# MILAB-IIT-CV/ATDN_vSLAM

Hardware: AMD Instinct MI355X
Metric: frame-pairs/sec, KITTI 1241x376 odometry inference at 1/2/4/8 MI355X (higher is better)
Workload: dtype f32 via 3xf16 split MFMA (fp32 accumulate); 1 GPU; KITTI seq-03-shaped 376x1241 uint8 frames (resident in HBM) resized to 376x1232, GMA flow 12 GRU iters + CLVO head -> 6-DoF trajectory (BASELINE configs[1]); streams_per_gpu=2, gru_iters=12, parallelism=pairs sharded x1, one all-gather of 512-d features, replicated LSTM scan

## Files before the change

### atdn_vslam_amd/csrc/gma.h

```cpp
#pragma once
#include <vector>
#include <map>
#include <memory>

#include "attention.h"
#include "conv_dispatch.h"
#include "device_buf.h"
#include "kernels.h"
#include "range_probe.h"
#include "weights.h"

namespace atdn {

struct EncoderWeights {
  PackedConv stem;
  struct Block { PackedConv c1, c2, ds; bool has_ds = false; } blk[6];
  PackedConv head;
};

class GmaNet {
 public:
  GmaNet(int H, int W, int max_batch, int precision);
  ~GmaNet();
  StateDict& state() { return sd_; }
// ... 11 lines not shown
  void profile(int B, int iters, int reps, float* ms, hipStream_t st, int mode = 0);

  int H, W, H8, W8, N, ldN, maxB, precision;
  int dev_ = 0;
  bool norm_on_load_ = false;
  bool classic_ = false;
  bool low_latency_ = false;
  void set_low_latency(bool on);
  DeviceBuf attn_part_;
  DeviceBuf enc2_[4];
  hipStream_t par_stream_ = nullptr;
  std::vector<hipEvent_t> par_events_;
  size_t par_next_ = 0;
  bool par_ = false;
  bool par_ok_ = true;
  void fork(hipStream_t from, hipStream_t to);
  DeviceBuf fbrick_[4], fplain_[3], coords_used_;
  DeviceBuf fpre_, fsrc_;
  PackedConv fhead_fold_;
  float corr_mul_ = 1.f;
  long fhead_w32_off_ = -1, fhead_b32_off_ = -1;
  int brickBW_[4], brickBH_[4], brickNB_[4];
  BrickPyramid brick_pyramid() const;
  DeviceBuf rowmax_, rinv_;

  struct ProbeRow { std::string name; int iter; bool limited; float max_abs; long long over, nonfinite; };
  static constexpr int kProbeMaxRows = 1536;
  void set_probe(bool on);
  const std::vector<ProbeRow>& probe_rows() const { return probe_rows_; }

 private:
  bool probe_ = false;
  int probe_it_ = -1;
  DeviceArray<RangeSlot> probe_slots_;
  std::vector<ProbeRow> probe_rows_;
  void probe_begin(hipStream_t st);
  void probe_end(hipStream_t st);
  void probe(const std::string& name, bool limited, const float* p, long rows, long cols, long ld, hipStream_t st);
  void run_body(int B, int iters, hipStream_t st);
  void run_encoder(const EncoderWeights& E, bool instance, int nimg, hipStream_t st, float** out_buf, int* outH,
                   int* outW);
  void iteration(int B, hipStream_t st);
  void run_body_sf(int B, int iters, hipStream_t st);
  void run_encoder_sf(const EncoderWeights& E, bool instance, int nimg, hipStream_t st, float** out_buf, int first_img = 0,
                      DeviceBuf* bufs = nullptr, float* final_dst = nullptr);
  void iteration_sf(int B, hipStream_t st);
  void capture(int B, int iters);
  void launch_body(int B, int iters, hipStream_t st);
  int seq_ = 0;
  int last_frame_ = -1;
  float* preds_out_ = nullptr;
  long preds_stride_ = 0;
  void mask_head_sf(int B, hipStream_t st);
  void mask_head(int B, hipStream_t st);
  int last_B_ = 0;

  StateDict sd_;
  WeightArena arena_;
  bool ready_ = false;
  bool use_graph_ = true;
  EncoderWeights fnet_, cnet_;
  PackedConv convc1_, convc2_, convf1_, convf2_, convm_, to_v_, to_qk_;
  long convf1_sf_off_ = -1;
  float convf1_wscale_ = 1.f;
  float fh2_mul_ = 1.f;
  long fh2_w32_off_ = -1;
  DeviceBuf fhG_;
  PackedConv gru_zr_[2], gru_q_[2], fh1_, fh2_, mask0_, mask2_;
  PackedConv gru_zr_ctx_[2], gru_q_ctx_[2];
  const float* gamma_ = nullptr;
  long gamma_off_ = -1;
  long to_v_w32_off_ = -1;

  DeviceBuf img4_, enc_[4], scratch_, pcnt_, fin_, fmap_ , psum_, pm2_, mean_[3], rstd_[3];
  DeviceBuf pyr_[4], h_[2], x_, qk_, attn_, vT_, corrfeat_, cor1_, corflo_, flo1_, z_, rh_, fh_, mask_;
  DeviceBuf coords1_, flow4_, pre_zr_[2], pre_q_[2];
  int pyrH_[4], pyrW_[4];
  size_t ws_bytes_ = 0;

  struct Timer;
  Timer* timer_ = nullptr;
  void mark(int stage, hipStream_t st);

  hipStream_t cap_stream_ = nullptr;
  std::map<std::pair<int, int>, hipGraphExec_t> graphs_;
};

}
```

### atdn_vslam_amd/csrc/gma.hip

```cpp
#include "gma.h"
#include "small_convs.h"
#include "conv_sf.h"
#include "epilogues_sf.h"

namespace atdn { const float* zero_line(); }

namespace atdn {

extern template TileChoice conv_dispatch<MODE_TAP, EpiBias<ACT_NONE>>(const ConvShape&, EpiBias<ACT_NONE>, hipStream_t);
extern template TileChoice conv_dispatch<MODE_TAP, EpiBias<ACT_RELU>>(const ConvShape&, EpiBias<ACT_RELU>, hipStream_t);
extern template TileChoice conv_dispatch<MODE_ROW, EpiBias<ACT_RELU>>(const ConvShape&, EpiBias<ACT_RELU>, hipStream_t);
extern template TileChoice conv_dispatch<MODE_TAP, EpiBiasStats>(const ConvShape&, EpiBiasStats, hipStream_t);
extern template TileChoice conv_dispatch<MODE_ROW, EpiBiasStats>(const ConvShape&, EpiBiasStats, hipStream_t);
extern template TileChoice conv_dispatch<MODE_TAP, EpiBiasReluAddRelu>(const ConvShape&, EpiBiasReluAddRelu, hipStream_t);
extern template TileChoice conv_dispatch<MODE_TAP, EpiContextSplit>(const ConvShape&, EpiContextSplit, hipStream_t);
extern template TileChoice conv_dispatch<MODE_TAP, EpiScale>(const ConvShape&, EpiScale, hipStream_t);
extern template TileChoice conv_dispatch<MODE_TAP, EpiQK>(const ConvShape&, EpiQK, hipStream_t);
extern template TileChoice conv_dispatch<MODE_TAP, EpiStoreT>(const ConvShape&, EpiStoreT, hipStream_t);
extern template TileChoice conv_dispatch<MODE_TAP, EpiAggregate>(const ConvShape&, EpiAggregate, hipStream_t);
extern template TileChoice conv_dispatch<MODE_TAP, EpiGruZR>(const ConvShape&, EpiGruZR, hipStream_t);
extern template TileChoice conv_dispatch<MODE_TAP, EpiGruQ>(const ConvShape&, EpiGruQ, hipStream_t);
extern template TileChoice conv_dispatch<MODE_TAP, EpiFlowDelta>(const ConvShape&, EpiFlowDelta, hipStream_t);

extern template TileChoice conv_dispatch<MODE_ROW, SfBias<ACT_RELU>>(const ConvShape&, SfBias<ACT_RELU>, hipStream_t);
// ... 202 lines not shown
    convf1_sf_off_ = arena_.alloc(4L * 2 * 4 * 2 * 64 * 4);
    _Float16* f = reinterpret_cast<_Float16*>(arena_.at(convf1_sf_off_));
    for (int wv = 0; wv < 4; ++wv)
      for (int cb = 0; cb < 2; ++cb)
        for (int s = 0; s < 4; ++s)
          for (int lane = 0; lane < 64; ++lane)
            for (int i = 0; i < 8; ++i) {
              const int n = 32 * wv + 16 * cb + (lane & 15), g = lane >> 4;
              const int ky = 2 * s + (g >> 1), kx = 4 * (g & 1) + (i >> 1), c = i & 1;
              const float v = (ky < 7 && kx < 7) ? std::ldexp(w.data[(((long)n * 2 + c) * 7 + ky) * 7 + kx], p) : 0.f;
              const _Float16 hi = (_Float16)v, lo = (_Float16)(v - (float)hi);
              const long frag = (((long)wv * 2 + cb) * 4 + s) * 2;
              f[(frag * 64 + lane) * 8 + i] = hi;
              f[((frag + 1) * 64 + lane) * 8 + i] = lo;
            }
  }
  convf2_ = tap({u + "encoder.convf2"});
  convm_ = tap({u + "encoder.conv"});
  to_v_ = tap({u + "aggregator.to_v"}, false);
  to_qk_ = tap({"att.to_qk"}, false);
  for (int p = 0; p < 2; ++p) {
    const std::string t = std::to_string(p + 1);
    if (sf) {
      const std::vector<std::pair<int, int>> ctx = {{128, 256}};
      const HostTensor& wv = sd_.get(u + "aggregator.to_v.weight");
      const HostTensor& gam = sd_.get(u + "aggregator.gamma");
      ATDN_CHECK(gam.data.size() == 1, "aggregator.gamma is one value");
      gru_zr_[p] = pack_gru_sf_folded(arena_, sd_, {u + "gru.convz" + t, u + "gru.convr" + t}, wv, (double)gam.data[0]);
      gru_q_[p] = pack_gru_sf_folded(arena_, sd_, {u + "gru.convq" + t}, wv, (double)gam.data[0]);
      gru_zr_ctx_[p] = pack_conv_sf_channels(arena_, sd_, {u + "gru.convz" + t, u + "gru.convr" + t}, ctx, false);
      gru_q_ctx_[p] = pack_conv_sf_channels(arena_, sd_, {u + "gru.convq" + t}, ctx, false);
    } else {
      gru_zr_[p] = tap({u + "gru.convz" + t, u + "gru.convr" + t});
      gru_q_[p] = tap({u + "gru.convq" + t});
    }
  }
  fh1_ = tap({u + "flow_head.conv1"});
  fh2_ = tap({u + "flow_head.conv2"});
  if (sf) {
    const HostTensor& w = sd_.get(u + "flow_head.conv2.weight");
    ATDN_CHECK(w.shape.size() == 4 && w.shape[0] == 2 && w.shape[1] == 256 && w.shape[2] == 3 && w.shape[3] == 3, "flow head conv2 shape");
    fh2_w32_off_ = arena_.alloc(18 * 256);
    for (int o = 0; o < 2; ++o)
      for (int c = 0; c < 256; ++c)
        for (int t = 0; t < 9; ++t) arena_.at(fh2_w32_off_)[(t * 2 + o) * 256 + c] = w.data[((long)o * 256 + c) * 9 + t];
    float mx = 0.f;
    for (float v : w.data) mx = std::max(mx, std::fabs(v));
    int e = 0;
    if (mx > 0.f) (void)std::frexp(mx, &e);
    fh2_mul_ = std::ldexp(1.0f, 1 - e);
  }
  mask0_ = tap({u + "mask.0"});
  mask2_ = tap({u + "mask.2"});
  gamma_off_ = pack_vector(arena_, sd_.get(u + "aggregator.gamma").data);
  if (sf) to_v_w32_off_ = pack_vector(arena_, sd_.get(u + "aggregator.to_v.weight").data);
  arena_.upload();
  resolve_encoder(arena_, fnet_);
  resolve_encoder(arena_, cnet_);
  for (PackedConv* L : {&convc1_, &convc2_, &convf1_, &convf2_, &convm_, &to_v_, &to_qk_, &gru_zr_[0], &gru_zr_[1],
                        &gru_q_[0], &gru_q_[1], &fh1_, &fh2_, &mask0_, &mask2_})
    resolve(arena_, *L);
  if (sf) for (PackedConv* L : {&gru_zr_ctx_[0], &gru_zr_ctx_[1], &gru_q_ctx_[0], &gru_q_ctx_[1], &fhead_fold_}) resolve(arena_, *L);
  gamma_ = arena_.dev(gamma_off_);

  const int B = maxB;
  const int H2 = conv_out(H, 7, 2, 3), W2 = conv_out(W, 7, 2, 3);
  const long n8 = (long)B * N;
  img4_.alloc(2L * B * H * W * 4);
  for (int i = 0; i < (sf ? 4 : 3); ++i) enc_[i].alloc(2L * B * H2 * W2 * 64);
  if (sf) { fpre_.alloc(2L * B * N * 128); fsrc_.alloc((long)B * N * 160); }
  else fmap_.alloc(2L * B * N * 256);
  const long groups = (long)cdiv(H2 * W2, 64) * 4 + 8;
  psum_.alloc(2L * B * groups * 128); pm2_.alloc(2L * B * groups * 128); pcnt_.alloc(2L * B * groups); fin_.alloc(2L * B * 32 * 128 * 4 * 2);
  for (int i = 0; i < 3; ++i) { mean_[i].alloc(2L * B * 128); rstd_[i].alloc(2L * B * 128); }
  pyrH_[0] = H8; pyrW_[0] = W8;
  for (int l = 1; l < 4; ++l) { pyrH_[l] = pyrH_[l - 1] / 2; pyrW_[l] = pyrW_[l - 1] / 2; }
  ATDN_CHECK(pyrH_[3] >= 2 && pyrW_[3] >= 2, "frame too small for a 4-level pyramid");
  for (int l = 0; l < 4; ++l) {
    brickBW_[l] = cdiv(pyrW_[l], 8); brickBH_[l] = cdiv(pyrH_[l], 4); brickNB_[l] = brickBW_[l] * brickBH_[l] * 32;
    pyr_[l].alloc(classic_ ? n8 * pyrH_[l] * pyrW_[l] : (long)B * brick_pixel_blocks(N) * kBrickPixelBlock * brickNB_[l]);
  }
  if (sf) {
    for (int l = 0; l < 4; ++l) fbrick_[l].alloc((long)B * brickNB_[l] * 160);
    for (int l = 1; l < 4; ++l) fplain_[l - 1].alloc((long)B * pyrH_[l] * pyrW_[l] * 128);
    coords_used_.alloc(n8 * 2);
  }
  h_[0].alloc(n8 * 128); h_[1].alloc(n8 * 128); x_.alloc(n8 * XLD);
  const AttnGeom ag = attn_geom(B, N, ldN);
  qk_.alloc(n8 * 256); attn_.alloc(std::max(n8 * ldN, attn_floats(ag)));
  if (classic_) vT_.alloc((long)B * 128 * ldN);
  if (sf) { rowmax_.alloc((long)B * ag.Npad); rinv_.alloc((long)B * ag.Npad); }
  if (sf && low_latency_ && attn_v_splits(attn_geom(1, N, ldN)) > 1) attn_part_.alloc(8L * B * ag.Npad * 128);
  if (sf && low_latency_) {
    for (int i = 0; i < 4; ++i) enc2_[i].alloc((long)B * H2 * W2 * 64);
    ATDN_HIP(hipStreamCreateWithFlags(&par_stream_, hipStreamNonBlocking));
    par_events_.resize(2 * (1 + 64));
    for (auto& e : par_events_) ATDN_HIP(hipEventCreateWithFlags(&e, hipEventDisableTiming));
  }
  corrfeat_.alloc(n8 * CORR_LD); cor1_.alloc(n8 * 256); corflo_.alloc(n8 * 256); flo1_.alloc(n8 * 128);
  z_.alloc(n8 * 128); rh_.alloc(n8 * 128); fh_.alloc(n8 * 256); mask_.alloc(n8 * 576);
  if (sf) fhG_.alloc(2 * n8 * 18);
  coords1_.alloc(n8 * 2); flow4_.alloc(n8 * 4);
  if (sf) for (int p = 0; p < 2; ++p) { pre_zr_[p].alloc(n8 * 256); pre_q_[p].alloc(n8 * 128); }
  ATDN_HIP(hipMemset(corrfeat_.p, 0, corrfeat_.n * sizeof(float)));
  if (vT_.p) ATDN_HIP(hipMemset(vT_.p, 0, vT_.n * sizeof(float)));
  ATDN_HIP(hipMemset(attn_.p, 0, attn_.n * sizeof(float)));
  ATDN_HIP(hipMemset(flow4_.p, 0, flow4_.n * sizeof(float)));
  ATDN_HIP(hipDeviceSynchronize());
  ws_bytes_ = 0;
  DeviceBuf* all[] = {&img4_, &enc_[0], &enc_[1], &enc_[2], &enc_[3], &fmap_, &fpre_, &fsrc_, &psum_, &pm2_, &pyr_[0], &pyr_[1], &pyr_[2],
                      &pyr_[3], &h_[0], &h_[1], &x_, &qk_, &attn_, &vT_, &corrfeat_, &cor1_, &corflo_, &flo1_, &z_,
                      &rh_, &fh_, &mask_, &coords1_, &flow4_};
  for (auto* b : all) ws_bytes_ += (size_t)b->n * sizeof(float);
  (void)zero_line();
  sf_counter_attach();
  ATDN_HIP(hipStreamCreateWithFlags(&cap_stream_, hipStreamNonBlocking));
  ready_ = true;
}

void GmaNet::run_encoder(const EncoderWeights& E, bool instance, int nimg, hipStream_t st, float** out_buf, int* outH,
                         int* outW) {
  int h = conv_out(H, 7, 2, 3), w = conv_out(W, 7, 2, 3);
  float* P = enc_[0].p; float* Q = enc_[1].p; float* R = enc_[2].p;
  auto stats_conv = [&](auto mode_tag, const PackedConv& L, const float* src, int ld, int ih, int iw, int stride,
                        int pad, float* dst, int slot) {
    constexpr int MODE = decltype(mode_tag)::value;
    ConvShape s = conv_shape(L, src, ld, (long)ih * iw * ld, nimg, ih, iw, stride, pad, pad);
    const int oh = conv_out(ih, L.KH, stride, pad), ow = conv_out(iw, L.KW, stride, pad);
    EpiBiasStats ep{L.b, dst, (long)oh * ow * L.N, L.N, psum_.p, pm2_.p, 0};
    TileChoice t = conv_dispatch<MODE>(s, ep, st);
    const int groups = cdiv(oh * ow, t.BM) * (t.BM / 32);
    ATDN_CHECK((long)nimg * groups * L.N <= psum_.n, "statistics scratch too small");
    launch_in_finalize_cnt(psum_.p, pm2_.p, nullptr, nimg, groups, oh * ow, L.N, 1e-5f, mean_[slot].p, rstd_[slot].p,
                           reinterpret_cast<double*>(fin_.p), st);
  };
  using TapT = std::integral_constant<int, MODE_TAP>;
  using RowT = std::integral_constant<int, MODE_ROW>;
  auto pr = [&](int bi, const char* leaf, bool limited, const float* p, long pixels, int ch) {
    if (!probe_) return;
    std::string name = instance ? "fnet." : "cnet.";
    if (bi >= 0) name += "layer" + std::to_string(bi / 2 + 1) + "." + std::to_string(bi % 2);
    probe(name + leaf, limited, p, (long)nimg * pixels, ch, ch, st);
  };

  if (instance) {
    stats_conv(RowT{}, E.stem, img4_.p, 4, H, W, 2, 3, P, 0);
    pr(-1, "conv1.raw", false, P, (long)h * w, 64);
    launch_in_apply(P, mean_[0].p, rstd_[0].p, nullptr, nullptr, nullptr, nimg, (long)h * w, 64, st);
  } else {
    ConvShape s = conv_shape(E.stem, img4_.p, 4, (long)H * W * 4, nimg, H, W, 2, 3, 3);
    conv_dispatch<MODE_ROW>(s, EpiBias<ACT_RELU>{E.stem.b, P, (long)h * w * 64, 64, 1.f}, st);
  }
  pr(-1, "conv1.out", true, P, (long)h * w, 64);
// ... 324 lines not shown
  run_encoder_sf(fnet_, true, nfeat, st, &f, seq_ == 2 ? 1 : 0, nullptr, fpre_.p + (seq_ == 2 ? (long)N * 128 : 0));
  ConvShape s = conv_shape(fhead_fold_, fpre_.p, 128, (long)N * 128, B, H8, W8, 1, 0, 0);
  conv_sf_dispatch(s, fhead_fold_.wscale, SfBias<ACT_NONE>{fhead_fold_.b, fsrc_.p, (long)N * 160, 160}, st);
  mark(ST_FNET, st);

  const float* target = fpre_.p + (long)(seq_ ? 1 : B) * N * 128;
  for (int l = 0; l < 4; ++l) {
    const float* plain = target;
    long plain_sb = (long)N * 128;
    if (l > 0) {
      const float* prev = l == 1 ? target : fplain_[l - 2].p;
      const long prev_sb = l == 1 ? (long)N * 128 : (long)pyrH_[l - 1] * pyrW_[l - 1] * 128;
      plain_sb = (long)pyrH_[l] * pyrW_[l] * 128;
      launch_pool_features_sf(prev, B, pyrH_[l - 1], pyrW_[l - 1], 128, prev_sb, fplain_[l - 1].p, plain_sb, st);
      plain = fplain_[l - 1].p;
    }
    launch_brick_rows(plain, plain_sb, B, pyrH_[l], pyrW_[l], 128, 160, fbrick_[l].p, (long)brickNB_[l] * 160, st);
    launch_corr_bricks(fsrc_.p, (long)N * 160, fbrick_[l].p, (long)brickNB_[l] * 160, B, N, brickNB_[l], 160,
                       corr_mul_ / sqrtf(256.0f), pyr_[l].p, sf_fast_mode(), st);
    if (l == 0) mark(ST_CORR, st);
  }
  mark(ST_POOL, st);

  run_encoder_sf(cnet_, false, B, sB, &f, 0, par_ ? enc2_ : nullptr);
  s = conv_shape(cnet_.head, f, 128, (long)N * 128, B, H8, W8, 1, 0, 0);
  conv_sf_dispatch(s, cnet_.head.wscale,
                   SfContextSplit{cnet_.head.b, h_[0].p, (long)N * 128, x_.p, (long)N * XLD, XLD}, sB);
  mark(ST_CNET, st);

  s = conv_shape(to_qk_, x_.p, XLD, (long)N * XLD, B, H8, W8, 1, 0, 0);
  conv_sf_dispatch(s, to_qk_.wscale, SfQK{1.0f / sqrtf(128.0f), 128, qk_.p, (long)N * 256, 256}, sB);
  {
    const AttnGeom ag = attn_geom(B, N, ldN);
    launch_qk_rowmax(qk_.p, ag, rowmax_.p, sB);
    mark(ST_ATTN_LOGITS, st);
    launch_qk_softmax(qk_.p, ag, rowmax_.p, attn_.p, rinv_.p, sf_fast_mode(), sB);
  }
  mark(ST_ATTN, st);

  for (int p = 0; p < 2; ++p) {
    const int ph = p ? 2 : 0, pw = p ? 0 : 2;
    ConvShape g = conv_shape(gru_zr_ctx_[p], x_.p, XLD, (long)N * XLD, B, H8, W8, 1, ph, pw);
    conv_sf_dispatch(g, gru_zr_ctx_[p].wscale, EpiBias<ACT_NONE>{nullptr, pre_zr_[p].p, (long)N * 256, 256, 1.f}, sB);
    g = conv_shape(gru_q_ctx_[p], x_.p, XLD, (long)N * XLD, B, H8, W8, 1, ph, pw);
    conv_sf_dispatch(g, gru_q_ctx_[p].wscale, EpiBias<ACT_NONE>{nullptr, pre_q_[p].p, (long)N * 128, 128, 1.f}, sB);
  }
  mark(ST_GRU_CTX, st);
  if (par_) fork(sB, st);

  for (int it = 0; it < iters; ++it) {
    iteration_sf(B, st);
    if (preds_out_) {
      mask_head_sf(B, st);
      launch_upsample(mask_.p, flow4_.p, B, H8, W8, nullptr, preds_out_ + it * preds_stride_, st);
    }
  }
  if (!preds_out_) mask_head_sf(B, st);
  mark(ST_MASK, st);
}

void GmaNet::mask_head_sf(int B, hipStream_t st) {
  ConvShape s = conv_shape(mask0_, h_[0].p, 128, (long)N * 128, B, H8, W8, 1, 1, 1);
  conv_sf_dispatch(s, mask0_.wscale, SfBias<ACT_RELU>{mask0_.b, fh_.p, (long)N * 256, 256}, st);
  s = conv_shape(mask2_, fh_.p, 256, (long)N * 256, B, H8, W8, 1, 0, 0);
  conv_sf_dispatch(s, mask2_.wscale, EpiBias<ACT_NONE>{mask2_.b, mask_.p, (long)N * 576, 576, 0.25f}, st);
}

void GmaNet::capture(int B, int iters) {
  const bool want_par = low_latency_ && precision >= 1 && B <= 2 && par_stream_ != nullptr && !preds_out_ && par_ok_;
  for (int attempt = want_par ? 0 : 1; attempt < 2; ++attempt) {
    hipGraph_t graph = nullptr;
    hipGraphExec_t exec = nullptr;
    ATDN_HIP(hipStreamBeginCapture(cap_stream_, hipStreamCaptureModeThreadLocal));
    par_ = attempt == 0;
    par_next_ = 0;
    try {
      if (precision >= 1) { FastGuard fg(precision == 2); run_body_sf(B, iters, cap_stream_); } else run_body(B, iters, cap_stream_);
      par_ = false;
      ATDN_HIP(hipStreamEndCapture(cap_stream_, &graph));
      ATDN_HIP(hipGraphInstantiate(&exec, graph, nullptr, nullptr, 0));
    } catch (...) {
      const bool was_par = par_ || attempt == 0;
      par_ = false;
      hipGraph_t g2 = nullptr;
      (void)hipStreamEndCapture(cap_stream_, &g2);
      if (g2) (void)hipGraphDestroy(g2);
      if (graph) (void)hipGraphDestroy(graph);
      (void)hipGetLastError();
      if (attempt == 0 && was_par) {
        fprintf(stderr, "atdn: the flow graph could not be captured with parallel branches; capturing it as one chain\n");
        par_ok_ = false;
        continue;
      }
      throw;
    }
    (void)hipGraphDestroy(graph);
    graphs_[{B, iters * 4 + seq_}] = exec;
    return;
  }
}

void GmaNet::forward_sequence(const float* frames, int B, int iters, const float* flow_init, float* flow_low,
                               float* flow_up, hipStream_t st, bool continued) {
  ATDN_CHECK(ready_, "weights not finalized");
  ATDN_CHECK(precision >= 1, "sequence mode is built for the split-f16 pipeline");
  ATDN_CHECK(B >= 1 && B <= maxB, "batch exceeds max_batch of this handle");
  ATDN_CHECK(iters >= 1 && iters <= 64, "iters out of range");
  ATDN_CHECK(frames && flow_low && flow_up, "null tensor");
  const long frame = 3L * H * W;
  if (continued) {
    ATDN_CHECK(last_frame_ >= 1, "continued sequence call without a previous sequence call on this handle");
    ATDN_HIP(hipMemcpyAsync(fpre_.p, fpre_.p + (long)last_frame_ * N * 128, (size_t)N * 128 * sizeof(float),
                            hipMemcpyDeviceToDevice, st));
    seq_ = 2;
  } else {
    seq_ = 1;
  }
  last_frame_ = 0;
  launch_prep_images(frames, frames + (long)B * frame, B, H, W, img4_.p, st, 1);
  launch_init_coords_sf(flow_init, B, H8, W8, coords1_.p, flow4_.p, x_.p, XLD, 254, st);
  launch_body(B, iters, st);
  launch_upsample(mask_.p, flow4_.p, B, H8, W8, flow_low, flow_up, st);
  last_frame_ = B;
}

void GmaNet::launch_body(int B, int iters, hipStream_t st) {
  last_B_ = B;
  if (use_graph_ && !probe_) {
    auto key = std::make_pair(B, iters * 4 + seq_);
    if (!graphs_.count(key)) capture(B, iters);
    ATDN_HIP(hipGraphLaunch(graphs_[key], st));
  } else {
    if (precision >= 1) { FastGuard fg(precision == 2); run_body_sf(B, iters, st); } else run_body(B, iters, st);
  }
}

void GmaNet::forward(const float* im1, const float* im2, int B, int iters, const float* flow_init, float* flow_low,
                     float* flow_up, hipStream_t st) {
  ATDN_CHECK(ready_, "weights not finalized");
  ATDN_CHECK(B >= 1 && B <= maxB, "batch exceeds max_batch of this handle");
  ATDN_CHECK(iters >= 1 && iters <= 64, "iters out of range");
  ATDN_CHECK(im1 && im2 && flow_low && flow_up, "null tensor");
  seq_ = 0;
  last_frame_ = 0;
  if (probe_) probe_begin(st);
  launch_prep_images(im1, im2, B, H, W, img4_.p, st, B);
  if (precision >= 1) launch_init_coords_sf(flow_init, B, H8, W8, coords1_.p, flow4_.p, x_.p, XLD, 254, st);
  else launch_init_coords(flow_init, B, H8, W8, coords1_.p, flow4_.p, x_.p + 254, XLD, st);
  if (probe_) {
    probe("image", true, img4_.p, 2L * B * H * W, 3, 4, st);
    probe("flow_init", true, flow4_.p, (long)B * N, 2, 4, st);
  }
  launch_body(B, iters, st);
  launch_upsample(mask_.p, flow4_.p, B, H8, W8, flow_low, flow_up, st);
  if (probe_) {
    probe("flow_low", false, flow_low, 1, 2L * B * N, 2L * B * N, st);
    probe("flow_up", false, flow_up, 1, 2L * B * H * W, 2L * B * H * W, st);
    probe_end(st);
  }
}

void GmaNet::forward_predictions(const float* im1, const float* im2, int B, int iters, const float* flow_init, float* preds,
                                 hipStream_t st) {
  ATDN_CHECK(ready_, "weights not finalized");
  ATDN_CHECK(B >= 1 && B <= maxB, "batch exceeds max_batch of this handle");
  ATDN_CHECK(iters >= 1 && iters <= 64, "iters out of range");
  ATDN_CHECK(im1 && im2 && preds, "null tensor");
  seq_ = 0;
  last_frame_ = 0;
  last_B_ = B;
  if (probe_) probe_begin(st);
  launch_prep_images(im1, im2, B, H, W, img4_.p, st, B);
  if (precision >= 1) launch_init_coords_sf(flow_init, B, H8, W8, coords1_.p, flow4_.p, x_.p, XLD, 254, st);
  else launch_init_coords(flow_init, B, H8, W8, coords1_.p, flow4_.p, x_.p + 254, XLD, st);
  if (probe_) {
    probe("image", true, img4_.p, 2L * B * H * W, 3, 4, st);
    probe("flow_init", true, flow4_.p, (long)B * N, 2, 4, st);
  }
  struct Guard {
    GmaNet* n; ~Guard() { n->preds_out_ = nullptr; n->preds_stride_ = 0; }
  } guard{this};
  preds_out_ = preds;
  preds_stride_ = (long)B * 2 * H * W;
  if (precision >= 1) { FastGuard fg(precision == 2); run_body_sf(B, iters, st); } else run_body(B, iters, st);
  if (probe_) probe_end(st);
}

BrickPyramid GmaNet::brick_pyramid() const {
  BrickPyramid bp;
  for (int l = 0; l < 4; ++l) {
    bp.base[l] = pyr_[l].p; bp.H[l] = pyrH_[l]; bp.W[l] = pyrW_[l];
    bp.BW[l] = brickBW_[l]; bp.BH[l] = brickBH_[l]; bp.NB[l] = brickNB_[l];
  }
  bp.N = N; bp.NPB = brick_pixel_blocks(N);
  return bp;
}

long GmaNet::debug_read(const char* name, float* host, long capacity, hipStream_t st) {
  const std::string k(name);
  if (!classic_ && k.size() == 4 && k.compare(0, 3, "pyr") == 0 && k[3] >= '0' && k[3] <= '3') {
    const int l = k[3] - '0';
    const long rows = (long)maxB * N, total = rows * pyrH_[l] * pyrW_[l];
    scratch_.reserve(total);
    launch_unbrick(pyr_[l].p, brickNB_[l], N, pyrH_[l], pyrW_[l], rows, scratch_.p, st);
    ATDN_HIP(hipStreamSynchronize(st));
    const long n = std::min(capacity, total);
    ATDN_HIP(hipMemcpy(host, scratch_.p, (size_t)n * sizeof(float), hipMemcpyDeviceToHost));
    return n;
  }
  if (!classic_ && k == "corrfeat") {
    launch_lookup_bricks(brick_pyramid(), coords_used_.p, (long)(last_B_ > 0 ? last_B_ : maxB) * N, corrfeat_.p, st);
  }
  if (k == "sf_clamped") {
    ATDN_CHECK(capacity >= 1, "sf_clamped needs room for one float");
    host[0] = (float)sf_counter_read_reset(st);
    return 1;
  }
  const DeviceBuf* b = nullptr;
  if (k == "fmap") b = &fmap_; else if (k == "pyr0") b = &pyr_[0]; else if (k == "pyr1") b = &pyr_[1];
  else if (k == "pyr2") b = &pyr_[2]; else if (k == "pyr3") b = &pyr_[3]; else if (k == "net") b = &h_[0];
  else if (k == "x") b = &x_; else if (k == "attn") b = &attn_; else if (k == "corrfeat") b = &corrfeat_;
  else if (k == "mask") b = &mask_; else if (k == "coords1") b = &coords1_; else if (k == "flow4") b = &flow4_;
  else if (k == "qk") b = &qk_; else if (k == "img4") b = &img4_;
  else if (k == "cor1") b = &cor1_;
  if (k == "fmap" && !classic_) {
    const long rows = 2L * maxB * N;
    scratch_.reserve(rows * (128 + 256));
    launch_from_sf(fpre_.p, scratch_.p, rows, 128, st);
    launch_linear_rows(scratch_.p, rows, 128, arena_.dev(fhead_w32_off_), arena_.dev(fhead_b32_off_), 256, scratch_.p + rows * 128, st);
    ATDN_HIP(hipStreamSynchronize(st));
    const long n = std::min(capacity, rows * 256);
    ATDN_HIP(hipMemcpy(host, scratch_.p + rows * 128, (size_t)n * sizeof(float), hipMemcpyDeviceToHost));
    return n;
  }
  if (k == "agg") {
    if (classic_) return -1;
    scratch_.reserve(x_.n);
    launch_from_sf(x_.p, scratch_.p, x_.n / 32, 32, st);
    ATDN_HIP(hipStreamSynchronize(st));
    const long rows = std::min(capacity / 128, (long)maxB * N);
    if (rows > 0)
      ATDN_HIP(hipMemcpy2D(host, 128 * sizeof(float), scratch_.p + 256, XLD * sizeof(float), 128 * sizeof(float), (size_t)rows,
                           hipMemcpyDeviceToHost));
    return rows * 128;
  }
  if (!b) return -1;
  long n = std::min(capacity, b->n);
  if (k == "attn" && !classic_) {
    const long rows = (long)maxB * N * ldN;
    scratch_.reserve(rows);
    ATDN_HIP(hipMemsetAsync(scratch_.p, 0, (size_t)rows * sizeof(float), st));
    launch_attn_decode(attn_.p, rinv_.p, attn_geom(maxB, N, ldN), scratch_.p, st);
    ATDN_HIP(hipStreamSynchronize(st));
    n = std::min(capacity, rows);
    ATDN_HIP(hipMemcpy(host, scratch_.p, (size_t)n * sizeof(float), hipMemcpyDeviceToHost));
    return n;
  }
  const bool is_sf = precision >= 1 && (k == "fmap" || k == "net" || k == "x" || k == "attn" || k == "corrfeat" || k == "qk" || k == "cor1");
  const float* src = b->p;
  if (is_sf) {
    scratch_.reserve(b->n);
    launch_from_sf(b->p, scratch_.p, b->n / 32, 32, st);
    src = scratch_.p;
    if (k == "x")
      launch_mfg_reconstruct(scratch_.p, (long)maxB * N, XLD, 128, 256, arena_.dev(to_v_w32_off_), gamma_, coords_used_.p, N, W8, 254, st);
// ... 8 lines not shown
```

### atdn_vslam_amd/csrc/kernels.h

```cpp
#pragma once
#include "common.h"

namespace atdn {

bool& sf_fast_mode();

struct PyramidLevels {
  const float* base[4];
  int H[4], W[4];
};

void launch_prep_images(const float* im1, const float* im2, int B, int H, int W, float* img4, hipStream_t st, int n2);

int stem_sf_groups(int Ho, int Wo);
void launch_stem_sf(int mode, const float* img4, int nimg, int H, int W, const float* wfrag, float wscale,
                    const float* bias, float* out_sf, float* part_sum, float* part_m2, float* part_cnt,
                    const float* mean, const float* rstd, hipStream_t st);

void launch_in_finalize_cnt(const float* part_sum, const float* part_m2, const float* part_cnt, int nimg,
                            int groups_per_img, int HW, int C, float eps, float* mean, float* rstd, double* scratch,
                            hipStream_t st);
void launch_in_apply(float* x, const float* mean, const float* rstd, const float* res, const float* rmean,
                     const float* rrstd, int nimg, long HW, int C, hipStream_t st);

void launch_avgpool(const float* src, int H, int W, float* dst, long rows, hipStream_t st);

void launch_lookup(const PyramidLevels& pyr, const float* coords1, long npix_total, float* out, int ldo,
                   hipStream_t st);

void launch_softmax_rows(float* x, long rows, int n, int ld, hipStream_t st);

void launch_init_coords(const float* flow_init, int B, int H8, int W8, float* coords1, float* flow4, float* xflow,
                        int ldx, hipStream_t st);

void launch_upsample(const float* mask, const float* flow4, int B, int H8, int W8, float* flow_low, float* flow_up,
                     hipStream_t st);

void launch_prep_flow(const float* flow, int B, int H, int W, const float* dw_w, const float* dw_b, float* out4,
                      hipStream_t st);
void launch_prep_rgb(const float* images, int B, int H, int W, float* out4, hipStream_t st);
void launch_linear(const float* W0, const float* x0, int K0, int ldx0, const float* W1, const float* x1, int K1,
                   int ldx1, const float* b0, const float* b1, int act, float* y, int ldy, int N, int B,
                   hipStream_t st);
struct LstmPipeArgs {
  int Hd, B, do1, do_lin, do2;
  const float *pre1, *Whh1, *bhh1, *h1_in; float *c1, *h1_out;
  const float *Wlin, *blin, *lin_in; float* lin_out;
  const float *Wih2, *bih2, *Whh2, *bhh2, *x2_in, *h2_in; float *c2, *h2_out;
};
void launch_lstm_pipe(const LstmPipeArgs& a, hipStream_t st);
long lstm_scan_exchange_bytes();
bool lstm_scan_fits_device();
void launch_lstm_scan(const float* pre1, const float* Whh1, const float* bhh1, const float* Wlin, const float* blin,
                      const float* Wih2, const float* bih2, const float* Whh2, const float* bhh2, float* state, float* h2seq,
                      void* exchange, int T, hipStream_t st);
struct MlpHead { const float *w0, *b0, *w1, *b1, *w2; };
void launch_mlp_heads(const float* h2, int B, MlpHead rot, MlpHead tr, float* rot_out, float* tr_out, hipStream_t st);

void launch_to_sf(const float* src, float* dst, long rows, int C, hipStream_t st);
void launch_from_sf(const float* src, float* dst, long rows, int C, hipStream_t st);
void launch_mfg_reconstruct(float* x, long rows, int ld, int cmf, int cagg, const float* wv, const float* gamma,
                            const float* coords_used, int N, int W8, int cflow, hipStream_t st);
void launch_in_apply_sf(const float* x, float* y, const float* mean, const float* rstd, const float* res,
                        const float* res_raw, const float* rmean, const float* rrstd, int nimg, long HW, int C,
                        hipStream_t st, bool res_relu = false);
void launch_pool_features_sf(const float* src, int nimg, int H, int W, int C, long sb, float* dst, long db, hipStream_t st);
void launch_init_coords_sf(const float* flow_init, int B, int H8, int W8, float* coords1, float* flow4, float* x,
                           int ldx, int cflow, hipStream_t st);

void launch_fill(float* p, long n, float v, hipStream_t st);

constexpr int kBrickPixelBlock = 64;
struct BrickPyramid {
  const float* base[4];
  int H[4], W[4], BW[4], BH[4], NB[4];
  int N;
  int NPB;
};
inline int brick_pixel_blocks(int N) { return 2 * ((N + 127) / 128); }
void launch_brick_rows(const float* src, long sb, int nimg, int H, int W, int C, int Cd, float* dst, long db, hipStream_t st);
void launch_corr_bricks(const float* f1, long sb1, const float* f2b, long sb2, int B, int N, int NB, int K, float scale,
                        float* out, bool fast, hipStream_t st);
void launch_linear_rows(const float* in, long rows, int Cin, const float* w, const float* b, int Cout, float* out, hipStream_t st);
void launch_unbrick(const float* src, long NB, int N, int H, int W, long npix, float* dst, hipStream_t st);
void launch_lookup_conv(const BrickPyramid& pyr, const float* coords1, long npix, float* coords_used, const float* wfrag,
                        float wscale, const float* bias, float* out, bool fast, hipStream_t st);
void launch_lookup_bricks(const BrickPyramid& pyr, const float* coords1, long npix, float* out, hipStream_t st);

}
// ... 1 lines not shown
```

### atdn_vslam_amd/csrc/weights.h

```cpp
#pragma once
#include <algorithm>
#include <cmath>
#include <cstring>
#include <map>
#include <string>
#include <vector>

#include "conv_mfma.h"
#include "device_buf.h"

namespace atdn {

struct HostTensor {
  std::vector<int64_t> shape;
  std::vector<float> data;
  long numel() const { long n = 1; for (auto d : shape) n *= d; return n; }
};

class StateDict {
 public:
  void put(const std::string& key, const float* data, const int64_t* shape, int rank) {
    std::string k = key;
    if (k.rfind("module.", 0) == 0) k = k.substr(7);
    HostTensor t;
// ... 74 lines not shown
  ATDN_CHECK(w0.shape.size() == 4, "conv weight must be 4-d");
  const int Cin = (int)w0.shape[1], KH = (int)w0.shape[2], KW = (int)w0.shape[3];
  L.mode = mode; L.KH = KH; L.KW = KW;
  L.C = (mode == MODE_TAP) ? round_up(Cin, 32) : Cpix;
  ATDN_CHECK(L.C >= Cin, "channel padding smaller than Cin");
  L.ldw = packed_k(mode, KH, KW, L.C);
  int N = 0;
  for (auto& nm : names) N += (int)sd.get(nm + ".weight").shape[0];
  L.N = N;
  L.w_off = A.alloc((long)N * L.ldw);
  L.b_off = A.alloc(N);
  int n0 = 0;
  for (auto& nm : names) {
    const HostTensor& w = sd.get(nm + ".weight");
    ATDN_CHECK((int)w.shape[1] == Cin && (int)w.shape[2] == KH && (int)w.shape[3] == KW, "stacked convs must agree");
    const int Co = (int)w.shape[0];
    const float* bias = (has_bias && sd.has(nm + ".bias")) ? sd.get(nm + ".bias").data.data() : nullptr;
    for (int n = 0; n < Co; ++n) {
      const double sc = fold ? fold->scale[n0 + n] : 1.0;
      float* row = A.at(L.w_off + (long)(n0 + n) * L.ldw);
      for (int c = 0; c < Cin; ++c)
        for (int ky = 0; ky < KH; ++ky)
          for (int kx = 0; kx < KW; ++kx) {
            const double v = (double)w.data[(((long)n * Cin + c) * KH + ky) * KW + kx] * sc;
            const long k = (mode == MODE_TAP) ? ((long)(ky * KW + kx) * L.C + c)
                                              : ((long)ky * round_up(KW * L.C, 32) + kx * L.C + c);
            row[k] = (float)v;
          }
      double bv = bias ? (double)bias[n] : 0.0;
      if (fold) bv = bv * sc + fold->shift[n0 + n];
      A.at(L.b_off)[n0 + n] = (float)bv;
    }
    n0 += Co;
  }
  return L;
}

inline void pack_fragment_major16(WeightArena& A, PackedConv& L) {
  const int nq = L.ldw / 32, nblk = (L.N + 15) / 16;
  L.wf16_off = A.alloc((long)nblk * nq * 512);
  const float* w = A.at(L.w_off);
  float* f = A.at(L.wf16_off);
  for (int nb = 0; nb < nblk; ++nb)
    for (int q = 0; q < nq; ++q)
      for (int hl = 0; hl < 2; ++hl)
        for (int lane = 0; lane < 64; ++lane) {
          const int r = lane & 15, gq = lane >> 4, row = nb * 16 + r, slot = 4 * hl + gq;
          float* d = f + ((((long)nb * nq + q) * 2 + hl) * 64 + lane) * 4;
          if (row < L.N) std::memcpy(d, w + (long)row * L.ldw + q * 32 + slot * 4, 16);
          else std::memset(d, 0, 16);
        }
}

inline PackedConv pack_conv_sf(WeightArena& A, const StateDict& sd, const std::vector<std::string>& names,
                               const ChannelAffine* fold = nullptr, bool has_bias = true) {
  PackedConv L = pack_conv(A, sd, names, MODE_TAP, 0, fold, has_bias);
  float* w = A.at(L.w_off);
  const long total = (long)L.N * L.ldw;
  float mx = 0.f;
  for (long i = 0; i < total; ++i) mx = std::max(mx, std::fabs(w[i]));
  int e = 0;
  if (mx > 0.f) (void)std::frexp(mx, &e);
  const int p = 1 - e;
  L.wscale = std::ldexp(1.0f, -p);
  std::vector<float> row(L.ldw);
  for (int n = 0; n < L.N; ++n) {
    float* r = w + (long)n * L.ldw;
    std::memcpy(row.data(), r, L.ldw * sizeof(float));
    _Float16* hrow = reinterpret_cast<_Float16*>(r);
    for (int q = 0; q < L.ldw / 32; ++q)
      for (int j = 0; j < 32; ++j) {
        const float v = std::ldexp(row[q * 32 + j], p);
        const _Float16 hi = (_Float16)v;
        const _Float16 lo = (_Float16)(v - (float)hi);
        hrow[q * 64 + j] = hi;
        hrow[q * 64 + 32 + j] = lo;
      }
  }
  if ((L.KH == 3 && L.KW == 3) || (L.KH == 1 && L.KW == 5) || (L.KH == 5 && L.KW == 1)) {
    pack_fragment_major16(A, L);
  }
  return L;
}

inline void pack_stem_sf(WeightArena& A, PackedConv& L) {
  ATDN_CHECK(L.mode == MODE_ROW && L.KH == 7 && L.KW == 7 && L.C == 4 && L.ldw == 224 && L.N == 64, "stem shape");
  L.wf_off = A.alloc(2L * 14 * 2 * 256);
  const float* w = A.at(L.w_off);
  float mx = 0.f;
  for (long i = 0; i < (long)L.N * L.ldw; ++i) mx = std::max(mx, std::fabs(w[i]));
  int e = 0;
  if (mx > 0.f) (void)std::frexp(mx, &e);
  const int p = 1 - e;
  L.wscale = std::ldexp(1.0f, -p);
  _Float16* f = reinterpret_cast<_Float16*>(A.at(L.wf_off));
  for (int nt = 0; nt < 2; ++nt)
    for (int q = 0; q < 14; ++q)
      for (int lane = 0; lane < 64; ++lane) {
        const int r = lane & 31, h = lane >> 5;
        for (int m = 0; m < 8; ++m) {
          const float v = std::ldexp(w[(long)(nt * 32 + r) * L.ldw + 16 * q + 8 * h + m], p);
          const _Float16 hi = (_Float16)v;
          f[(((long)(nt * 14 + q) * 2 + 0) * 64 + lane) * 8 + m] = hi;
          f[(((long)(nt * 14 + q) * 2 + 1) * 64 + lane) * 8 + m] = (_Float16)(v - (float)hi);
        }
      }
// ... 133 lines not shown
```

Before: 447.6 frame-pairs/s.

## Fuse mask conv2 with convex upsampling into one MFMA kernel

Replaces the separate 1x1 mask.2 conv (which wrote a 576-channel mask to HBM) and the upsample kernel with a single kernel. It computes the mask logits via split-f16 MFMA in registers, applies the softmax over the 9 neighbours, and writes the upsampled flow directly. This removes the large mask write and read and one launch per forward. The cost is a bespoke kernel with heavy register use and special weight packing, and debug reads now recompute the stored mask on demand.

```diff
diff --git a/atdn_vslam_amd/csrc/gma.h b/atdn_vslam_amd/csrc/gma.h
--- a/atdn_vslam_amd/csrc/gma.h
+++ b/atdn_vslam_amd/csrc/gma.h
@@ -87,6 +87,8 @@
   float* preds_out_ = nullptr;
   long preds_stride_ = 0;
   void mask_head_sf(int B, hipStream_t st);
+  void upsample_sf(int B, float* flow_low, float* flow_up, hipStream_t st);
+  void mask2_stored_sf(int B, float* dst, hipStream_t st);
   void mask_head(int B, hipStream_t st);
   int last_B_ = 0;
 
diff --git a/atdn_vslam_amd/csrc/gma.hip b/atdn_vslam_amd/csrc/gma.hip
--- a/atdn_vslam_amd/csrc/gma.hip
+++ b/atdn_vslam_amd/csrc/gma.hip
@@ -278,6 +278,7 @@
   }
   mask0_ = tap({u + "mask.0"});
   mask2_ = tap({u + "mask.2"});
+  if (sf) pack_mask_upsample_fragments(arena_, mask2_);
   gamma_off_ = pack_vector(arena_, sd_.get(u + "aggregator.gamma").data);
   if (sf) to_v_w32_off_ = pack_vector(arena_, sd_.get(u + "aggregator.to_v.weight").data);
   arena_.upload();
@@ -324,7 +325,8 @@
     for (auto& e : par_events_) ATDN_HIP(hipEventCreateWithFlags(&e, hipEventDisableTiming));
   }
   corrfeat_.alloc(n8 * CORR_LD); cor1_.alloc(n8 * 256); corflo_.alloc(n8 * 256); flo1_.alloc(n8 * 128);
-  z_.alloc(n8 * 128); rh_.alloc(n8 * 128); fh_.alloc(n8 * 256); mask_.alloc(n8 * 576);
+  z_.alloc(n8 * 128); rh_.alloc(n8 * 128); fh_.alloc(n8 * 256);
+  if (classic_) mask_.alloc(n8 * 576);
   if (sf) fhG_.alloc(2 * n8 * 18);
   coords1_.alloc(n8 * 2); flow4_.alloc(n8 * 4);
   if (sf) for (int p = 0; p < 2; ++p) { pre_zr_[p].alloc(n8 * 256); pre_q_[p].alloc(n8 * 128); }
@@ -755,7 +757,7 @@
     iteration_sf(B, st);
     if (preds_out_) {
       mask_head_sf(B, st);
-      launch_upsample(mask_.p, flow4_.p, B, H8, W8, nullptr, preds_out_ + it * preds_stride_, st);
+      upsample_sf(B, nullptr, preds_out_ + it * preds_stride_, st);
     }
   }
   if (!preds_out_) mask_head_sf(B, st);
@@ -765,8 +767,16 @@
 void GmaNet::mask_head_sf(int B, hipStream_t st) {
   ConvShape s = conv_shape(mask0_, h_[0].p, 128, (long)N * 128, B, H8, W8, 1, 1, 1);
   conv_sf_dispatch(s, mask0_.wscale, SfBias<ACT_RELU>{mask0_.b, fh_.p, (long)N * 256, 256}, st);
-  s = conv_shape(mask2_, fh_.p, 256, (long)N * 256, B, H8, W8, 1, 0, 0);
-  conv_sf_dispatch(s, mask2_.wscale, EpiBias<ACT_NONE>{mask2_.b, mask_.p, (long)N * 576, 576, 0.25f}, st);
+}
+
+void GmaNet::upsample_sf(int B, float* flow_low, float* flow_up, hipStream_t st) {
+  launch_mask_upsample(fh_.p, mask2_.wf16, mask2_.wscale, mask2_.b, flow4_.p, B, H8, W8, flow_low, flow_up, precision == 2, st);
+}
+
+void GmaNet::mask2_stored_sf(int B, float* dst, hipStream_t st) {
+  FastGuard fg(precision == 2);
+  ConvShape s = conv_shape(mask2_, fh_.p, 256, (long)N * 256, B, H8, W8, 1, 0, 0);
+  conv_sf_dispatch(s, mask2_.wscale, EpiBias<ACT_NONE>{mask2_.b, dst, (long)N * 576, 576, 0.25f}, st);
 }
 
 void GmaNet::capture(int B, int iters) {
@@ -823,7 +833,7 @@
   launch_prep_images(frames, frames + (long)B * frame, B, H, W, img4_.p, st, 1);
   launch_init_coords_sf(flow_init, B, H8, W8, coords1_.p, flow4_.p, x_.p, XLD, 254, st);
   launch_body(B, iters, st);
-  launch_upsample(mask_.p, flow4_.p, B, H8, W8, flow_low, flow_up, st);
+  upsample_sf(B, flow_low, flow_up, st);
   last_frame_ = B;
 }
 
@@ -855,7 +865,8 @@
     probe("flow_init", true, flow4_.p, (long)B * N, 2, 4, st);
   }
   launch_body(B, iters, st);
-  launch_upsample(mask_.p, flow4_.p, B, H8, W8, flow_low, flow_up, st);
+  if (classic_) launch_upsample(mask_.p, flow4_.p, B, H8, W8, flow_low, flow_up, st);
+  else upsample_sf(B, flow_low, flow_up, st);
   if (probe_) {
     probe("flow_low", false, flow_low, 1, 2L * B * N, 2L * B * N, st);
     probe("flow_up", false, flow_up, 1, 2L * B * H * W, 2L * B * H * W, st);
@@ -914,6 +925,24 @@
   if (!classic_ && k == "corrfeat") {
     launch_lookup_bricks(brick_pyramid(), coords_used_.p, (long)(last_B_ > 0 ? last_B_ : maxB) * N, corrfeat_.p, st);
   }
+  if (!classic_ && (k == "mask" || k == "flow_up_stored" || k == "flow_low_stored")) {
+    const int Bl = last_B_ > 0 ? last_B_ : maxB;
+    const long nmask = (long)maxB * N * 576, nup = (long)Bl * 2 * H * W, nlow = (long)Bl * 2 * N;
+    scratch_.reserve(nmask + nup + nlow);
+    ATDN_HIP(hipMemsetAsync(scratch_.p, 0, (size_t)nmask * sizeof(float), st));
+    mask2_stored_sf(Bl, scratch_.p, st);
+    const float* src = scratch_.p;
+    long total = nmask;
+    if (k != "mask") {
+      launch_upsample(scratch_.p, flow4_.p, Bl, H8, W8, scratch_.p + nmask + nup, scratch_.p + nmask, st);
+      src = k == "flow_up_stored" ? scratch_.p + nmask : scratch_.p + nmask + nup;
+      total = k == "flow_up_stored" ? nup : nlow;
+    }
+    ATDN_HIP(hipStreamSynchronize(st));
+    const long n = std::min(capacity, total);
+    ATDN_HIP(hipMemcpy(host, src, (size_t)n * sizeof(float), hipMemcpyDeviceToHost));
+    return n;
+  }
   if (k == "sf_clamped") {
     ATDN_CHECK(capacity >= 1, "sf_clamped needs room for one float");
     host[0] = (float)sf_counter_read_reset(st);
diff --git a/atdn_vslam_amd/csrc/kernels.h b/atdn_vslam_amd/csrc/kernels.h
--- a/atdn_vslam_amd/csrc/kernels.h
+++ b/atdn_vslam_amd/csrc/kernels.h
@@ -35,6 +35,8 @@
 
 void launch_upsample(const float* mask, const float* flow4, int B, int H8, int W8, float* flow_low, float* flow_up,
                      hipStream_t st);
+void launch_mask_upsample(const float* fh, const float* wfrag, float wscale, const float* bias, const float* flow4, int B,
+                          int H8, int W8, float* flow_low, float* flow_up, bool fast, hipStream_t st);
 
 void launch_prep_flow(const float* flow, int B, int H, int W, const float* dw_w, const float* dw_b, float* out4,
                       hipStream_t st);
diff --git a/atdn_vslam_amd/csrc/mask_upsample.hip b/atdn_vslam_amd/csrc/mask_upsample.hip
--- /dev/null
+++ b/atdn_vslam_amd/csrc/mask_upsample.hip
@@ -0,0 +1,201 @@
+#include "kernels.h"
+#include "sf.h"
+
+namespace atdn {
+
+namespace {
+
+constexpr int MU_NWM = 2;
+constexpr int MU_PIX = 64 * MU_NWM;
+constexpr int MU_THREADS = 256 * MU_NWM;
+constexpr int MU_ROWF = 40;
+constexpr int MU_IMG = MU_PIX * MU_ROWF;
+constexpr int MU_SLAB = 2 * MU_IMG / (4 * MU_NWM);
+constexpr int MU_PLANE = 264;
+static_assert(4 * MU_PLANE <= MU_SLAB, "a half-wave's four planes fit its slab");
+
+typedef float f32x4v __attribute__((ext_vector_type(4)));
+
+template <bool FAST>
+__global__ __launch_bounds__(MU_THREADS) void mask_upsample_kernel(const float* __restrict__ fh, const float* __restrict__ wfrag,
+                                                                   const float wscale, const float* __restrict__ bias,
+                                                                   const float* __restrict__ flow4, const int H8, const int W8,
+                                                                   const int tiles, float* __restrict__ flow_low,
+                                                                   float* __restrict__ flow_up) {
+  extern __shared__ __attribute__((aligned(16))) float lds[];
+  const int tid = threadIdx.x, lane = tid & 63, wave = tid >> 6;
+  const int wm = wave >> 2, wg = wave & 3;
+  const int N = H8 * W8;
+  const int img = blockIdx.x / tiles;
+  const int pix0 = (blockIdx.x - img * tiles) * MU_PIX;
+  const float4* f4 = reinterpret_cast<const float4*>(flow4) + (long)img * N;
+
+  if (flow_low && tid < MU_PIX && pix0 + tid < N) {
+    const float4 f = f4[pix0 + tid];
+    flow_low[((long)img * 2 + 0) * N + pix0 + tid] = f.x;
+    flow_low[((long)img * 2 + 1) * N + pix0 + tid] = f.y;
+  }
+
+  const int SL = MU_PIX + 2 * W8 + 2;
+  float2* strip = reinterpret_cast<float2*>(lds + 2 * MU_IMG);
+  for (int idx = tid; idx < SL; idx += MU_THREADS) {
+    const int p = pix0 - W8 - 1 + idx;
+    const bool in = (unsigned)p < (unsigned)N;
+    const float4 f = f4[in ? p : 0];
+    const float2 v = make_float2(in ? 8.f * f.x : 0.f, in ? 8.f * f.y : 0.f);
+    const int w = in ? p % W8 : 1;
+    strip[idx] = w == W8 - 1 ? make_float2(0.f, 0.f) : v;
+    strip[SL + idx] = v;
+    strip[2 * SL + idx] = w == 0 ? make_float2(0.f, 0.f) : v;
+  }
+
+  const int s = tid & 7, r0 = tid >> 3;
+  const float* src[2];
+  bool ok[2];
+#pragma unroll
+  for (int i = 0; i < 2; ++i) {
+    const int m = pix0 + r0 + MU_PIX / 2 * i;
+    ok[i] = m < N;
+    src[i] = fh + ((long)img * N + (ok[i] ? m : 0)) * 256 + 4 * s;
+  }
+  float4 ra[2];
+  auto fetch = [&](int q) __attribute__((always_inline)) {
+#pragma unroll
+    for (int i = 0; i < 2; ++i) ra[i] = *reinterpret_cast<const float4*>(src[i] + q * 32);
+  };
+  auto stage = [&](int q) __attribute__((always_inline)) {
+#pragma unroll
+    for (int i = 0; i < 2; ++i)
+      *reinterpret_cast<float4*>(lds + (q & 1) * MU_IMG + (r0 + MU_PIX / 2 * i) * MU_ROWF + 4 * s) = keep_if(ok[i], ra[i]);
+  };
+
+  const char* wb = reinterpret_cast<const char*>(wfrag) + (long)wg * (72 * 2048) + lane * 16;
+  f16x8 bh[3], bl[3];
+  auto loadw = [&](int j, int slot) __attribute__((always_inline)) {
+    bh[slot] = *reinterpret_cast<const f16x8*>(wb + j * 2048);
+    if constexpr (!FAST) bl[slot] = *reinterpret_cast<const f16x8*>(wb + j * 2048 + 1024);
+  };
+
+  f32x4v acc[4][9];
+#pragma unroll
+  for (int i = 0; i < 4; ++i)
+#pragma unroll
+    for (int t = 0; t < 9; ++t)
+#pragma unroll
+      for (int e = 0; e < 4; ++e) acc[i][t][e] = 0.f;
+
+  fetch(0);
+  loadw(0, 0);
+  loadw(1, 1);
+  stage(0);
+  __syncthreads();
+
+  const int rr = lane & 15, hh = lane >> 4;
+  const char* a_rd = reinterpret_cast<const char*>(lds + (wm * 64 + rr) * MU_ROWF) + 16 * hh;
+#pragma unroll 1
+  for (int q = 0; q < 8; ++q) {
+    fetch(min(q + 1, 7));
+    const char* ap = a_rd + (q & 1) * (MU_IMG * 4);
+    f16x8 ah[4], al[4];
+#pragma unroll
+    for (int i = 0; i < 4; ++i) {
+      ah[i] = *reinterpret_cast<const f16x8*>(ap + i * 16 * (MU_ROWF * 4));
+      if constexpr (!FAST) al[i] = *reinterpret_cast<const f16x8*>(ap + i * 16 * (MU_ROWF * 4) + 64);
+    }
+    __builtin_amdgcn_sched_barrier(0);
+#pragma unroll
+    for (int t = 0; t < 9; ++t) {
+      loadw(min(q * 9 + t + 2, 71), (t + 2) % 3);
+      __builtin_amdgcn_sched_barrier(0);
+#pragma unroll
+      for (int i = 0; i < 4; ++i) {
+        f32x4v c = acc[i][t];
+        if constexpr (!FAST) {
+          c = __builtin_amdgcn_mfma_f32_16x16x32_f16(al[i], bh[t % 3], c, 0, 0, 0);
+          c = __builtin_amdgcn_mfma_f32_16x16x32_f16(ah[i], bl[t % 3], c, 0, 0, 0);
+        }
+        c = __builtin_amdgcn_mfma_f32_16x16x32_f16(ah[i], bh[t % 3], c, 0, 0, 0);
+        acc[i][t] = c;
+      }
+      __builtin_amdgcn_sched_barrier(0);
+    }
+    stage(q + 1);
+    __syncthreads();
+  }
+
+  const int n = lane & 15, g = lane >> 4;
+  float bs[9];
+#pragma unroll
+  for (int t = 0; t < 9; ++t) bs[t] = bias[t * 64 + wg * 16 + n];
+  float* slab = lds + wave * MU_SLAB;
+  const long Hf = 8L * H8, Wf = 8L * W8;
+#pragma unroll
+  for (int half = 0; half < 2; ++half) {
+#pragma unroll
+    for (int i2 = 0; i2 < 2; ++i2) {
+      const int i = half * 2 + i2;
+      const float2* nb = strip + wm * 64 + i * 16 + 4 * g;
+#pragma unroll
+      for (int el = 0; el < 4; ++el) {
+        float e[9];
+        float mx = -INFINITY;
+#pragma unroll
+        for (int k = 0; k < 9; ++k) {
+          const float v = acc[i][k][el] * wscale + bs[k];
+          e[k] = v * 0.25f;
+          mx = fmaxf(mx, e[k]);
+        }
+        float sum = 0.f;
+#pragma unroll
+        for (int k = 0; k < 9; ++k) { e[k] = __builtin_amdgcn_exp2f((e[k] - mx) * 1.4426950408889634f); sum += e[k]; }
+        const float rs = 1.0f / sum;
+        float ux = 0.f, uy = 0.f;
+#pragma unroll
+        for (int k = 0; k < 9; ++k) {
+          const float2 f = nb[(k % 3) * SL + (k / 3) * W8 + k % 3 + el];
+          const float wk = e[k] * rs;
+          ux += wk * f.x;
+          uy += wk * f.y;
+        }
+        float* d = slab + (n >> 3) * MU_PLANE + (i2 * 16 + 4 * g + el) * 8 + (n & 7);
+        d[0] = ux;
+        d[2 * MU_PLANE] = uy;
+      }
+    }
+    asm volatile("s_waitcnt lgkmcnt(0)" ::: "memory");
+    __builtin_amdgcn_wave_barrier();
+    const int m = pix0 + wm * 64 + half * 32 + (lane >> 1);
+    if (m < N) {
+      const int h = m / W8, w = m - h * W8;
+#pragma unroll
+      for (int c = 0; c < 2; ++c)
+#pragma unroll
+        for (int r = 0; r < 2; ++r) {
+          const float4 v = *reinterpret_cast<const float4*>(slab + (c * 2 + r) * MU_PLANE + 4 * lane);
+          float* o = flow_up + (((long)img * 2 + c) * Hf + 8 * h + 2 * wg + r) * Wf + 8 * w + 4 * (lane & 1);
+          *reinterpret_cast<float4*>(o) = v;
+        }
+    }
+    asm volatile("s_waitcnt lgkmcnt(0)" ::: "memory");
+    __builtin_amdgcn_wave_barrier();
+  }
+}
+
+}
+
+void launch_mask_upsample(const float* fh, const float* wfrag, float wscale, const float* bias, const float* flow4, int B,
+                          int H8, int W8, float* flow_low, float* flow_up, bool fast, hipStream_t st) {
+  const int tiles = cdiv(H8 * W8, MU_PIX);
+  const size_t lds_bytes = (size_t)2 * MU_IMG * sizeof(float) + (size_t)3 * (MU_PIX + 2 * W8 + 2) * sizeof(float2);
+  ATDN_CHECK(lds_bytes <= 160 * 1024, "map too wide for the upsampling kernel's flow strips (W / 8 <= 2495)");
+  auto launch = [&](auto kernel) {
+    if (lds_bytes > 64 * 1024)
+      ATDN_HIP(hipFuncSetAttribute(reinterpret_cast<const void*>(kernel), hipFuncAttributeMaxDynamicSharedMemorySize, 160 * 1024));
+    hipLaunchKernelGGL(kernel, dim3(B * tiles), dim3(MU_THREADS), lds_bytes, st, fh, wfrag, wscale, bias, flow4, H8, W8, tiles, flow_low,
+                       flow_up);
+  };
+  if (fast) launch(mask_upsample_kernel<true>); else launch(mask_upsample_kernel<false>);
+  ATDN_HIP(hipGetLastError());
+}
+
+}
diff --git a/atdn_vslam_amd/csrc/weights.h b/atdn_vslam_amd/csrc/weights.h
--- a/atdn_vslam_amd/csrc/weights.h
+++ b/atdn_vslam_amd/csrc/weights.h
@@ -150,6 +150,22 @@
         }
 }
 
+inline void pack_mask_upsample_fragments(WeightArena& A, PackedConv& L) {
+  ATDN_CHECK(L.N == 576 && L.ldw == 256 && L.KH == 1 && L.KW == 1, "mask2 shape");
+  L.wf16_off = A.alloc(4L * 72 * 512);
+  const float* w = A.at(L.w_off);
+  float* f = A.at(L.wf16_off);
+  for (int sg = 0; sg < 4; ++sg)
+    for (int q = 0; q < 8; ++q)
+      for (int t = 0; t < 9; ++t)
+        for (int hl = 0; hl < 2; ++hl)
+          for (int lane = 0; lane < 64; ++lane) {
+            const int r = lane & 15, gq = lane >> 4, row = t * 64 + sg * 16 + r, slot = 4 * hl + gq;
+            float* d = f + ((((long)sg * 72 + q * 9 + t) * 2 + hl) * 64 + lane) * 4;
+            std::memcpy(d, w + (long)row * L.ldw + q * 32 + slot * 4, 16);
+          }
+}
+
 inline PackedConv pack_conv_sf(WeightArena& A, const StateDict& sd, const std::vector<std::string>& names,
                                const ChannelAffine* fold = nullptr, bool has_bias = true) {
   PackedConv L = pack_conv(A, sd, names, MODE_TAP, 0, fold, has_bias);
```

Result: no change. 449.6 frame-pairs/s, median of 6 (+0.5%).
